# jdeschut/tunempc

Hardware: AMD Instinct MI355X
Metric: stage-Hessian convexifications/sec at (nx+nu)=32, p=64 (higher is better)
Workload: dtype f64

## Files before the change

tunempc_amd/csrc/tmpc_factor.h:

```cpp
#pragma once
#include "tmpc_common.h"

namespace tmpc {


#ifndef TMPC_LDP
#define TMPC_LDP 65
#endif
constexpr int FACT_LDS_DOUBLES = 2 * 64 * TMPC_LDP + 72 + 4 * 16 * 17 + 8;

enum { GM_SUB = 0, GM_SET = 1, GM_NEG = 2 };
constexpr int GM_NOTRI = -(1 << 30);

constexpr int SLD = 17, SUBD = 64 * SLD, SLABD = 2 * SUBD;
#ifdef TMPC_NT
#define TMPC_LD(p) __builtin_nontemporal_load(p)
#else
#define TMPC_LD(p) (*(p))
#endif
typedef const double __attribute__((address_space(1)))* gcptr;
typedef const double2_t __attribute__((address_space(1)))* gcptr2;
#define TMPC_LD4(dst, off, p, ok)                                                       \
  {                                                                                     \
    const double2_t u0_ = (ok) ? ((gcptr2)(p))[0] : (double2_t){0.0, 0.0};              \
    const double2_t u1_ = (ok) ? ((gcptr2)(p))[1] : (double2_t){0.0, 0.0};              \
    dst[(off) + 0] = u0_[0]; dst[(off) + 1] = u0_[1]; dst[(off) + 2] = u1_[0]; dst[(off) + 3] = u1_[1]; \
  }
#define TMPC_LD4F(dst, off, p, ok)                                                      \
  {                                                                                     \
    const float4_t u_ = (ok) ? *(const float4_t __attribute__((address_space(1)))*)(p) : (float4_t){0.f, 0.f, 0.f, 0.f}; \
    dst[(off) + 0] = (double)u_[0]; dst[(off) + 1] = (double)u_[1]; dst[(off) + 2] = (double)u_[2]; dst[(off) + 3] = (double)u_[3]; \
  }
typedef double __attribute__((address_space(1)))* gptr;
template <int WM, int WN, int FA, int NS = 2>
struct GemmCfg {
  static constexpr int TM = 16 * FA * WM, TN = 32 * WN, NTH = 64 * WM * WN, RP = NTH / 4;
  static constexpr int ARP = (TM + RP - 1) / RP, BRP = (TN + RP - 1) / RP;
  static constexpr int ASUB = TM * 17, BSUB = TN * 17, BUFD = NS * ASUB + NS * BSUB;
  static constexpr int LDS_DOUBLES = 2 * BUFD;
};

template <bool USE_MFMA, int WM = 2, int WN = 2, int FA = 2, int NS = 2>
__device__ __forceinline__ void wg_gemm_nt(double* C, int ldc, const double* A, int lda,
                                           const double* B, int ldb, int M, int N, int K, int mode, bool lower,
                                           double* lds) {
  typedef GemmCfg<WM, WN, FA, NS> G;
  constexpr int GKT = 16 * NS;
  constexpr int TM = G::TM, TN = G::TN, RP = G::RP, ARP = G::ARP, BRP = G::BRP, ASUB = G::ASUB, BSUB = G::BSUB, BUFD = G::BUFD;
  const int tid = threadIdx.x, lane = tid & 63, wv = tid >> 6;
  const int wr = wv / WN, wc = wv % WN;
  const int lrow = tid >> 2, lk = (tid & 3) * 4;
  const int nks = (K + GKT - 1) / GKT;
  const int fk = lane >> 4, fq = (lane >> 2) & 3, fj = lane & 3;
  const int wr0 = wr * 16 * FA, wc0 = wc * 32;
  constexpr bool CPRE = (FA <= 2) && (NS == 2);
  double acc[FA][8], cpre[CPRE ? FA : 1][8];
#pragma unroll
  for (int i = 0; i < FA; ++i)
#pragma unroll
    for (int j = 0; j < 8; ++j) { acc[i][j] = 0.0; if (CPRE) cpre[i][j] = 0.0; }
  double ra[ARP * 8], rb[BRP * 8];
  int m0 = 0, n0 = 0, ks = 0;
  const __amdgpu_buffer_rsrc_t arsrc = __builtin_amdgcn_make_buffer_rsrc((void*)A, 0, (int)(((unsigned)(M - 1) * (unsigned)lda + (unsigned)K) * 8u), 0x00020000);
  const __amdgpu_buffer_rsrc_t brsrc = __builtin_amdgcn_make_buffer_rsrc((void*)B, 0, (int)(((unsigned)(N - 1) * (unsigned)ldb + (unsigned)K) * 8u), 0x00020000);
  const unsigned avo = (unsigned)(lrow * lda + lk) * 8u, bvo = (unsigned)(lrow * ldb + lk) * 8u;
  typedef unsigned int u4_t __attribute__((ext_vector_type(4)));
#define TMPC_BLD4(dst, off, rsrc, vo, so)                                                                   \
  {                                                                                                         \
    const double2_t u0_ = __builtin_bit_cast(double2_t, __builtin_amdgcn_raw_buffer_load_b128(rsrc, (vo), (so), 0));          \
    const double2_t u1_ = __builtin_bit_cast(double2_t, __builtin_amdgcn_raw_buffer_load_b128(rsrc, (vo) + 16u, (so), 0));    \
    dst[(off) + 0] = u0_[0]; dst[(off) + 1] = u0_[1]; dst[(off) + 2] = u1_[0]; dst[(off) + 3] = u1_[1];    \
  }
#define TMPC_SLAB_LOAD(M0, N0, KN)                                                                          \
  {                                                                                                         \
    const unsigned aso = (unsigned)((M0) * lda + (KN) - lk) * 8u, bso = (unsigned)((N0) * ldb + (KN) - lk) * 8u;    \
    _Pragma("unroll") for (int rp = 0; rp < ARP; ++rp) {                                                    \
      if (RP * ARP == TM || lrow + rp * RP < TM) {                                                          \
        _Pragma("unroll") for (int h2 = 0; h2 < NS; ++h2)                                                   \
          TMPC_BLD4(ra, rp * 8 + h2 * 4, arsrc, avo + (unsigned)(rp * RP * lda + h2 * 16) * 8u, aso)        \
      }                                                                                                     \
    }                                                                                                       \
    _Pragma("unroll") for (int rp = 0; rp < BRP; ++rp) {                                                    \
      if (RP * BRP == TN || lrow + rp * RP < TN) {                                                          \
        _Pragma("unroll") for (int h2 = 0; h2 < NS; ++h2)                                                   \
          TMPC_BLD4(rb, rp * 8 + h2 * 4, brsrc, bvo + (unsigned)(rp * RP * ldb + h2 * 16) * 8u, bso)        \
      }                                                                                                     \
    }                                                                                                       \
  }
#define TMPC_SLAB_STORE(BUF)                                                                                \
  {                                                                                                         \
    double* An_ = lds + (BUF) * BUFD;                                                                       \
    double* Bn_ = An_ + NS * ASUB;                                                                           \
    _Pragma("unroll") for (int rp = 0; rp < ARP; ++rp) {                                                    \
      const int row = lrow + rp * RP;                                                                       \
      if (RP * ARP == TM || row < TM) {                                                                     \
        _Pragma("unroll") for (int h2 = 0; h2 < NS; ++h2)                                                   \
          _Pragma("unroll") for (int q = 0; q < 4; ++q) An_[h2 * ASUB + row * SLD + lk + q] = ra[rp * 8 + h2 * 4 + q]; \
      }                                                                                                     \
    }                                                                                                       \
    _Pragma("unroll") for (int rp = 0; rp < BRP; ++rp) {                                                    \
      const int row = lrow + rp * RP;                                                                       \
      if (RP * BRP == TN || row < TN) {                                                                     \
        _Pragma("unroll") for (int h2 = 0; h2 < NS; ++h2)                                                   \
          _Pragma("unroll") for (int q = 0; q < 4; ++q) Bn_[h2 * BSUB + row * SLD + lk + q] = rb[rp * 8 + h2 * 4 + q]; \
      }                                                                                                     \
    }                                                                                                       \
  }
  TMPC_SLAB_LOAD(0, 0, lk)
  __syncthreads();
  TMPC_SLAB_STORE(0)
  __syncthreads();
  int buf = 0;
  TMPC_T0()
  while (m0 < M) {
    int nm0 = m0, nn0 = n0, nks_ = ks + 1;
    if (nks_ == nks) {
      nks_ = 0; nn0 = n0 + TN;
      if (nn0 >= N || (lower && nn0 > nm0)) { nn0 = 0; nm0 = m0 + TM; }
    }
    const bool more = nm0 < M;
    if (more) TMPC_SLAB_LOAD(nm0, nn0, nks_ * GKT + lk)
    TMPC_T(0)
    const bool wave_on = (m0 + wr0 < M) && (n0 + wc0 < N) && !(lower && n0 == m0 && wc0 >= wr0 + 16 * FA);
    if (CPRE && ks == 0 && mode == GM_SUB && wave_on) {
#pragma unroll
      for (int i = 0; i < FA; ++i) {
        const int rbase = m0 + wr0 + i * 16;
#pragma unroll
        for (int m = 0; m < 2; ++m) {
          const int cbase = n0 + wc0 + m * 16;
          if (rbase < M && cbase < N) {
            gcptr2 cp2 = (gcptr2)(C + (size_t)(rbase + 4 * fq + fk) * ldc + cbase + 4 * fj);
            const double2_t u0 = cp2[0], u1 = cp2[1];
            cpre[CPRE ? i : 0][4 * m + 0] = u0[0]; cpre[CPRE ? i : 0][4 * m + 1] = u0[1]; cpre[CPRE ? i : 0][4 * m + 2] = u1[0]; cpre[CPRE ? i : 0][4 * m + 3] = u1[1];
          }
        }
      }
    }
    TMPC_T(1)
    if (wave_on) {
      const double* As = lds + buf * BUFD;
      const double* Bs = As + NS * ASUB;
      const int krem = K - ks * GKT;
      if (USE_MFMA) {
#define TMPC_MFMA_STEP(kk)                                                                              \
  {                                                                                                     \
    const int so = ((kk) & 3) * 4 + fk;                                                                 \
    const double* Ak = As + ((kk) >> 2) * ASUB + so;                                                    \
    const double* Bk = Bs + ((kk) >> 2) * BSUB + so;                                                    \
    double av[FA];                                                                                      \
    _Pragma("unroll") for (int i = 0; i < FA; ++i) av[i] = Ak[(wr0 + 16 * i + 4 * fq + fj) * SLD];       \
    _Pragma("unroll") for (int cb = 0; cb < 8; ++cb) {                                                  \
      const double bv = Bk[(wc0 + 16 * (cb >> 2) + 4 * fj + (cb & 3)) * SLD];                           \
      _Pragma("unroll") for (int i = 0; i < FA; ++i)                                                    \
        acc[i][cb] = __builtin_amdgcn_mfma_f64_4x4x4f64(av[i], bv, acc[i][cb], 0, 0, 0);                \
    }                                                                                                   \
  }
        if (NS == 1 || krem >= GKT) {
          if (FA <= 2) {
#pragma unroll
            for (int kk = 0; kk < GKT / 4; ++kk) TMPC_MFMA_STEP(kk)
          } else {
#pragma unroll 2
            for (int kk = 0; kk < GKT / 4; ++kk) TMPC_MFMA_STEP(kk)
          }
        } else {
          if (FA <= 2) {
#pragma unroll
            for (int kk = 0; kk < GKT / 8; ++kk) TMPC_MFMA_STEP(kk)
          } else {
#pragma unroll 2
            for (int kk = 0; kk < GKT / 8; ++kk) TMPC_MFMA_STEP(kk)
          }
        }
#undef TMPC_MFMA_STEP
      } else {
        const int kmax = (krem >= GKT) ? GKT : krem;
        for (int kk = 0; kk < kmax; ++kk) {
#pragma unroll
          for (int i = 0; i < FA; ++i)
#pragma unroll
            for (int cb = 0; cb < 8; ++cb) {
              const int row = wr0 + i * 16 + 4 * fq + fk, col = wc0 + 16 * (cb >> 2) + 4 * fj + (cb & 3);
              acc[i][cb] = fma(As[(kk >> 4) * ASUB + row * SLD + (kk & 15)], Bs[(kk >> 4) * BSUB + col * SLD + (kk & 15)], acc[i][cb]);
            }
        }
      }
    }
    TMPC_T(2)
    if (more) TMPC_SLAB_STORE(buf ^ 1)
    TMPC_T(3)
    if (ks == nks - 1 && wave_on) {
#pragma unroll
      for (int i = 0; i < FA; ++i) {
        const int rbase = m0 + wr0 + i * 16;
#pragma unroll
        for (int m = 0; m < 2; ++m) {
          const int cbase = n0 + wc0 + m * 16;
          if (rbase < M && cbase < N) {
            typedef double2_t __attribute__((address_space(1)))* gptr2;
            gptr2 cp2 = (gptr2)(C + (size_t)(rbase + 4 * fq + fk) * ldc + cbase + 4 * fj);
            double c0[4] = {0.0, 0.0, 0.0, 0.0};
            if (mode == GM_SUB) {
              if (CPRE) { c0[0] = cpre[CPRE ? i : 0][4 * m]; c0[1] = cpre[CPRE ? i : 0][4 * m + 1]; c0[2] = cpre[CPRE ? i : 0][4 * m + 2]; c0[3] = cpre[CPRE ? i : 0][4 * m + 3]; }
              else { const double2_t u0 = ((gcptr2)cp2)[0], u1 = ((gcptr2)cp2)[1]; c0[0] = u0[0]; c0[1] = u0[1]; c0[2] = u1[0]; c0[3] = u1[1]; }
            }
            double v[4];
#pragma unroll
            for (int e = 0; e < 4; ++e) {
              const double t = acc[i][4 * m + e];
              v[e] = (mode == GM_SUB) ? c0[e] - t : ((mode == GM_NEG) ? -t : t);
            }
            cp2[0] = (double2_t){v[0], v[1]}; cp2[1] = (double2_t){v[2], v[3]};
          }
#pragma unroll
          for (int e = 0; e < 4; ++e) acc[i][4 * m + e] = 0.0;
        }
      }
    }
    TMPC_T(4)
    __syncthreads();
    TMPC_T(5)
    buf ^= 1;
    m0 = nm0; n0 = nn0; ks = nks_;
  }
#undef TMPC_SLAB_LOAD
#undef TMPC_SLAB_STORE
#undef TMPC_BLD4
}

constexpr int LDP = TMPC_LDP;

__device__ __forceinline__ double potrf_rsqrt(double x) {
  double r = __builtin_amdgcn_rsq(x);
  r = r * (1.5 - 0.5 * x * r * r);
  r = r * (1.5 - 0.5 * x * r * r);
  return r;
}
template <int J>
__device__ __forceinline__ double row_bcast16(double v) { return __builtin_amdgcn_update_dpp(0.0, v, 0x150 + J, 0xF, 0xF, false); }
template <int K>
__device__ __forceinline__ void fmac_bcast16(double& acc, double x, double y) {
  asm volatile("s_nop 1\n\tv_fmac_f64_dpp %0, %1, %2 row_newbcast:%3 row_mask:0xf bank_mask:0xf" : "+v"(acc) : "v"(x), "v"(y), "n"(K));
}
struct Potrf16State { double a[16]; double m[4]; double nbad, minr, myref, thr8; int r, g; };
template <int J, int K>
__device__ __forceinline__ void potrf16_arow(Potrf16State& st, double nlj, double lj) {
  if constexpr (K < 16) { fmac_bcast16<K>(st.a[K], nlj, lj); potrf16_arow<J, K + 1>(st, nlj, lj); }
}
template <int J, int Q>
__device__ __forceinline__ void potrf16_mrow(Potrf16State& st, double fr) {
  if constexpr (Q <= J / 4) { fmac_bcast16<J>(st.m[Q], st.m[Q], fr); potrf16_mrow<J, Q + 1>(st, fr); }
}
template <int J>
__device__ __forceinline__ void potrf16_step(Potrf16State& st) {
  const double piv = row_bcast16<J>(st.a[J]);
  const double th8 = row_bcast16<J>(st.thr8);
  double rinv;
  {
    const double r0 = __builtin_amdgcn_rsq(piv);
    const double t = piv * r0, h = fma(-t, r0, 1.0);
    const double c = fma(0.375, h, 0.5), hc = h * c;
    rinv = fma(r0, hc, r0);
  }
  double lj = st.a[J] * rinv;
  if (__builtin_amdgcn_ballot_w64(!(piv > th8)) != 0) {
    const double ref = row_bcast16<J>(st.myref);
    if (piv < 1e-8 * ref) st.minr = fmin(st.minr, fmax(piv, 0.0) / ref);
    if (!(piv > 1e-15 * ref) || !(piv > 0.0)) {
      const double sub = (ref > 0.0 ? ref : 1.0) * 1e20;
      st.nbad += 1.0;
      rinv = potrf_rsqrt(sub);
      lj = (st.r == J) ? sub * rinv : st.a[J] * rinv;
    }
  }
  st.a[J] = lj;
  const double nlj = -lj;
  const double fr = (st.r > J) ? nlj * rinv : 0.0;
  potrf16_arow<J, J + 1>(st, nlj, lj);
  potrf16_mrow<J, 0>(st, fr);
  if constexpr (J + 1 < 16) potrf16_step<J + 1>(st);
}
template <int LDQ = LDP>
__device__ __forceinline__ void wave_potrf16(double* S, double* Si, const double* dr, double* stat, int lane) {
  Potrf16State st;
  st.r = lane & 15; st.g = lane >> 4;
#pragma unroll
  for (int k = 0; k < 16; ++k) st.a[k] = S[st.r * LDQ + k];
#pragma unroll
  for (int q = 0; q < 4; ++q) st.m[q] = (4 * q + st.g == st.r) ? 1.0 : 0.0;
  st.myref = fabs(dr[st.r]); st.thr8 = 1e-8 * st.myref;
  st.nbad = 0.0; st.minr = 1.0;
  __builtin_amdgcn_s_setprio(3);
  potrf16_step<0>(st);
  __builtin_amdgcn_s_setprio(0);
  if (lane < 16) {
#pragma unroll
    for (int k = 0; k < 16; ++k) if (k <= st.r) S[st.r * LDQ + k] = st.a[k];
  }
  wave_lds_sync();
  double myrinv;
  {
    const double d = S[st.r * LDQ + st.r];
    double x = __builtin_amdgcn_rcp(d);
    x = fma(fma(-d, x, 1.0), x, x);
    x = fma(fma(-d, x, 1.0), x, x);
    myrinv = x;
  }
#pragma unroll
  for (int q = 0; q < 4; ++q) { const int c = 4 * q + st.g; Si[st.r * LDQ + c] = (c <= st.r) ? st.m[q] * myrinv : 0.0; }
  if (lane == 0) { stat[0] += st.nbad; stat[1] = fmin(stat[1], st.minr); }
  wave_lds_sync();
}

__device__ __noinline__ int wg_potrf_inv(double* T, int ldt, double* Ti, const double* dref, int nb, double* lds, double* minr, double* stat = nullptr, int sw = 0, bool preloaded = false) {
  const int tid = threadIdx.x, lane = tid & 63, wv = tid >> 6;
  TMPC_TC0()
  double* S = lds;
  double* Si = S + 64 * LDP;
  double* dr = Si + 64 * LDP;
  double* tmp = dr + 72 + wv * (16 * 17);
  {
    const int i = tid >> 2, j0 = (tid & 3) * 16;
    double2_t v[8];
    const bool on = i < nb && j0 < nb;
    if (on && !preloaded) {
      gcptr2 src = (gcptr2)(T + (size_t)i * ldt + j0);
#pragma unroll
      for (int q = 0; q < 8; ++q) v[q] = src[q];
#pragma unroll
      for (int q = 0; q < 8; ++q) { S[i * LDP + j0 + 2 * q] = v[q][0]; S[i * LDP + j0 + 2 * q + 1] = v[q][1]; }
    }
    if (on) {
#pragma unroll
      for (int q = 0; q < 8; ++q) { Si[i * LDP + j0 + 2 * q] = 0.0; Si[i * LDP + j0 + 2 * q + 1] = 0.0; }
    }
  }
  if (tid < nb) dr[tid] = dref[tid];
  if (tid == 0) { dr[65] = 0.0; dr[66] = 1.0; }
  __syncthreads();
  const int nbk = nb >> 4;
  TMPC_TC(7, 0)
  for (int jb = 0; jb < nbk; ++jb) {
    const int o = 16 * jb;
    if (wv == sw) wave_potrf16(S + o * LDP + o, Si + o * LDP + o, dr + o, dr + 65, lane);
    __syncthreads();
    TMPC_TC(7, 1)
    {
      const int bi = jb + 1 + wv;
      if (bi < nbk) {
        double4_t acc = (double4_t){0.0, 0.0, 0.0, 0.0};
        acc = mm16(S + 16 * bi * LDP + o, LDP, Si + o * LDP + o, 1, LDP, acc, 1.0, lane);
        store_d16(S + 16 * bi * LDP + o, LDP, acc, lane);
      }
    }
    __syncthreads();
    {
      int q = 0;
      for (int bi = jb + 1; bi < nbk; ++bi)
        for (int bj = jb + 1; bj <= bi; ++bj, ++q)
          if ((q & 3) == wv) {
            double* Cp = S + 16 * bi * LDP + 16 * bj;
            double4_t acc = load_d16(Cp, LDP, lane);
            acc = mm16(S + 16 * bi * LDP + o, LDP, S + 16 * bj * LDP + o, 1, LDP, acc, -1.0, lane);
            store_d16(Cp, LDP, acc, lane);
          }
    }
    __syncthreads();
    TMPC_TC(7, 2)
  }
  for (int bi = 1; bi < nbk; ++bi) {
    const int bj = wv;
    if (bj < bi) {
      double4_t acc = (double4_t){0.0, 0.0, 0.0, 0.0};
      for (int k = bj; k < bi; ++k) acc = mm16(S + 16 * bi * LDP + 16 * k, LDP, Si + 16 * k * LDP + 16 * bj, LDP, 1, acc, 1.0, lane);
      store_d16(tmp, 17, acc, lane);
      wave_lds_sync();
      double4_t r = (double4_t){0.0, 0.0, 0.0, 0.0};
      r = mm16(Si + 16 * bi * LDP + 16 * bi, LDP, tmp, 17, 1, r, -1.0, lane);
      store_d16(Si + 16 * bi * LDP + 16 * bj, LDP, r, lane);
    }
    __syncthreads();
  }
  TMPC_TC(7, 3)
  {
    const int i = tid >> 2, j0 = (tid & 3) * 16;
    if (i < nb && j0 < nb) {
      typedef double2_t __attribute__((address_space(1)))* gptr2;
      gptr2 dt = (gptr2)(T + (size_t)i * ldt + j0);
      gptr2 di = (gptr2)(Ti + i * TB + j0);
#pragma unroll
      for (int q = 0; q < 8; ++q) {
        const int j = j0 + 2 * q;
        di[q] = (double2_t){Si[i * LDP + j], Si[i * LDP + j + 1]};
        if (j + 1 <= i) dt[q] = (double2_t){S[i * LDP + j], S[i * LDP + j + 1]};
        else if (j <= i) T[(size_t)i * ldt + j] = S[i * LDP + j];
      }
    }
  }
  __syncthreads();
  TMPC_TC(7, 4)
  const int nb_bad = (int)dr[65];
  if (stat) { if (tid == 0) { stat[0] += dr[65]; stat[1] = fmin(stat[1], dr[66]); } }
  else *minr = fmin(*minr, dr[66]);
  __syncthreads();
  return nb_bad;
}

template <bool USE_MFMA>
__device__ __forceinline__ int wg_block_column(double* Dk, double* R1, double* R2, double* Linv_k, const double* dref,
                                               int dp, double* lds, double* minr) {
  int nbad = 0;
  int jt = 0;
  TMPC_TC0()
  for (int j0 = 0; j0 < dp; j0 += TB, ++jt) {
    const int nb = (dp - j0 < TB) ? dp - j0 : TB;
    if (j0 > 0) {
      wg_gemm_nt<USE_MFMA>(Dk + (size_t)j0 * dp + j0, dp, Dk + (size_t)j0 * dp, dp, Dk + (size_t)j0 * dp, dp, dp - j0, nb, j0, GM_SUB, false, lds);
      if (R1) wg_gemm_nt<USE_MFMA>(R1 + j0, dp, R1, dp, Dk + (size_t)j0 * dp, dp, dp, nb, j0, GM_SUB, false, lds);
      if (R2) wg_gemm_nt<USE_MFMA>(R2 + j0, dp, R2, dp, Dk + (size_t)j0 * dp, dp, dp, nb, j0, GM_SUB, false, lds);
    }
    TMPC_TC(6, 0)
    double* Ti = Linv_k + (size_t)jt * TB * TB;
    nbad += wg_potrf_inv(Dk + (size_t)j0 * dp + j0, dp, Ti, dref + j0, nb, lds, minr);
    TMPC_TC(6, 1)
    if (dp - j0 - nb > 0)
      wg_gemm_nt<USE_MFMA>(Dk + (size_t)(j0 + nb) * dp + j0, dp, Dk + (size_t)(j0 + nb) * dp + j0, dp, Ti, TB, dp - j0 - nb, nb, nb, GM_SET, false, lds);
    if (R1) wg_gemm_nt<USE_MFMA>(R1 + j0, dp, R1 + j0, dp, Ti, TB, dp, nb, nb, GM_SET, false, lds);
    if (R2) wg_gemm_nt<USE_MFMA>(R2 + j0, dp, R2 + j0, dp, Ti, TB, dp, nb, nb, GM_SET, false, lds);
    TMPC_TC(6, 2)
  }
  return nbad;
}

constexpr int NCP = 4;
constexpr int GKV = 16, GLDV = GKV + 1;

template <bool TRANS, bool LOWER = false, typename MT = double>
__device__ __forceinline__ void wg_gemv16(double* Y, int yld, const double* X, int xld, const MT* M, int ldm,
                                          int rows, int cols, bool accumulate, double sgn, double* As, int nc) {
  constexpr bool F32 = sizeof(MT) == 4;
  const int tid = threadIdx.x, lane = tid & 63, wv = tid >> 6;
  const int fr = lane & 15, fk = lane >> 4;
  const int nks = cols / GKV;
  for (int m0 = 0; m0 < rows; m0 += 64) {
    double4_t acc = (double4_t){0.0, 0.0, 0.0, 0.0};
    double ra[4];
    const int lrow = TRANS ? (tid >> 4) : (tid >> 2);
    const int lcol = TRANS ? ((tid & 15) * 4) : ((tid & 3) * 4);
    const bool ok = TRANS ? (m0 + lcol < rows) : (m0 + lrow < rows);
    const MT* src = TRANS ? (M + (size_t)lrow * ldm + m0 + lcol) : (M + (size_t)(m0 + lrow) * ldm + lcol);
    const size_t kstep = TRANS ? (size_t)GKV * ldm : (size_t)GKV;
    double rb[4], rc[4], rd[4];
#define TMPC_GEMV_OK(KS) (ok && (!LOWER || (TRANS ? (m0 + lcol <= GKV * (KS) + lrow) : (GKV * (KS) + lcol <= m0 + lrow))))
#define TMPC_GEMV_LD(RG, P, OK) { if (F32) TMPC_LD4F(RG, 0, P, OK) else TMPC_LD4(RG, 0, P, OK) }
    TMPC_GEMV_LD(ra, src, TMPC_GEMV_OK(0))
    if (nks > 1) { const MT* s1 = src + kstep; TMPC_GEMV_LD(rb, s1, TMPC_GEMV_OK(1)) }
    if (nks > 2) { const MT* s1 = src + 2 * kstep; TMPC_GEMV_LD(rc, s1, TMPC_GEMV_OK(2)) }
    if (nks > 3) { const MT* s1 = src + 3 * kstep; TMPC_GEMV_LD(rd, s1, TMPC_GEMV_OK(3)) }
#define TMPC_GEMV_SLAB(RG, KS)                                                                                  \
    {                                                                                                             \
      __syncthreads();                                                                                            \
      if (TRANS) {                                                                                                \
        _Pragma("unroll") for (int q = 0; q < 4; ++q) As[(lcol + q) * GLDV + lrow] = RG[q];                     \
      } else {                                                                                                    \
        _Pragma("unroll") for (int q = 0; q < 4; ++q) As[lrow * GLDV + lcol + q] = RG[q];                       \
      }                                                                                                           \
      __syncthreads();                                                                                            \
      if ((KS) + 4 < nks) {                                                                                       \
        const MT* s2 = src + (size_t)((KS) + 4) * kstep;                                                          \
        TMPC_GEMV_LD(RG, s2, TMPC_GEMV_OK((KS) + 4))                                                             \
      }                                                                                                           \
      if (m0 + 16 * wv < rows) {                                                                                  \
        const int k0 = (KS) * GKV;                                                                                \
        _Pragma("unroll") for (int kk = 0; kk < GKV / 4; ++kk) {                                                 \
          const double a = As[(16 * wv + fr) * GLDV + kk * 4 + fk];                                               \
          const double bq = X[(fr & (NCP - 1)) * xld + k0 + kk * 4 + fk];                                         \
          acc = __builtin_amdgcn_mfma_f64_16x16x4f64(a, bq, acc, 0, 0, 0);                                        \
        }                                                                                                         \
      }                                                                                                           \
    }
    for (int ks = 0; ks < nks; ks += 4) {
      TMPC_GEMV_SLAB(ra, ks)
      if (ks + 1 < nks) TMPC_GEMV_SLAB(rb, ks + 1)
      if (ks + 2 < nks) TMPC_GEMV_SLAB(rc, ks + 2)
      if (ks + 3 < nks) TMPC_GEMV_SLAB(rd, ks + 3)
    }
#undef TMPC_GEMV_SLAB
#undef TMPC_GEMV_LD
#undef TMPC_GEMV_OK
    if (m0 + 16 * wv < rows && fr < nc) {
#pragma unroll
      for (int r = 0; r < 4; ++r) {
        const int i = m0 + 16 * wv + fk + 4 * r;
        if (i < rows) {
          double* yp = Y + fr * yld + i;
          *yp = (accumulate ? *yp : 0.0) + sgn * acc[r];
        }
      }
    }
  }
  __syncthreads();
}

__device__ __forceinline__ void blk_fwd(double* z, int xld, double* tmp, int tld, const double* Dk, const double* Lik, int dp,
                                        double* As, int nc) {
  int jt = 0;
  for (int j0 = 0; j0 < dp; j0 += TB, ++jt) {
    const int nb = (dp - j0 < TB) ? dp - j0 : TB;
    const double* Ti = Lik + (size_t)jt * TB * TB;
    wg_gemv16<false, true>(tmp, tld, z + j0, xld, Ti, TB, nb, nb, false, 1.0, As, nc);
    for (int e = threadIdx.x; e < nb * nc; e += 256) { const int q = e / nb, i = e - q * nb; z[q * xld + j0 + i] = tmp[q * tld + i]; }
    __syncthreads();
    const int rem = dp - j0 - nb;
    if (rem > 0) wg_gemv16<false>(z + j0 + nb, xld, z + j0, xld, Dk + (size_t)(j0 + nb) * dp + j0, dp, rem, nb, true, -1.0, As, nc);
  }
}
__device__ __forceinline__ void blk_bwd(double* z, int xld, double* tmp, int tld, const double* Dk, const double* Lik, int dp,
                                        double* As, int nc) {
  const int nt = (dp + TB - 1) / TB;
  for (int jt = nt - 1; jt >= 0; --jt) {
    const int j0 = jt * TB;
    const int nb = (dp - j0 < TB) ? dp - j0 : TB;
    const double* Ti = Lik + (size_t)jt * TB * TB;
    wg_gemv16<true, true>(tmp, tld, z + j0, xld, Ti, TB, nb, nb, false, 1.0, As, nc);
    for (int e = threadIdx.x; e < nb * nc; e += 256) { const int q = e / nb, i = e - q * nb; z[q * xld + j0 + i] = tmp[q * tld + i]; }
    __syncthreads();
    if (j0 > 0) wg_gemv16<true>(z, xld, z + j0, xld, Dk + (size_t)j0 * dp, dp, j0, nb, true, -1.0, As, nc);
  }
}

__device__ __forceinline__ void vec_g2s(double* z, int xld, const double* R, int dp, int nc) {
  for (int e = threadIdx.x; e < dp * nc; e += 256) { const int i = e / nc, q = e - i * nc; z[q * xld + i] = R[e]; }
}
__device__ __forceinline__ void vec_s2g(double* R, const double* z, int xld, int dp, int nc) {
  for (int e = threadIdx.x; e < dp * nc; e += 256) { const int i = e / nc, q = e - i * nc; R[e] = z[q * xld + i]; }
}

template <int NTH = 256>
__device__ __forceinline__ double wg_reduce_sum(double v, double* red) {
  const int lane = threadIdx.x & 63, wv = threadIdx.x >> 6;
  for (int o = 32; o > 0; o >>= 1) v += __shfl_xor(v, o, 64);
  __syncthreads();
  if (lane == 0) red[wv] = v;
  __syncthreads();
  double r = red[0];
#pragma unroll
  for (int q = 1; q < NTH / 64; ++q) r += red[q];
  __syncthreads();
  return r;
}

template <int NTH>
__device__ __forceinline__ void solve_border_body(const WS& w, const Dims& dm, int b, int pass, double* red) {
  const int* ip = w.iprob + (size_t)b * IS;
  const int phase = ip[I_PHASE];
  if (phase == PH_DONE) return;
  double* pr = w.prob + (size_t)b * PS;
  const int p = dm.p, dp = dm.dp, tid = threadIdx.x, nx = dm.nx;
  const size_t vl = (size_t)p * dp;
  double* W3 = w.W3 + (size_t)b * vl * 3;
  double* Z = w.Z + (size_t)b * vl;
  double* TU = w.TU + (size_t)b * vl * 2;
  const double* U = w.U + (size_t)b * vl * 2;
  if (pass == 1 && phase != PH_MAIN) return;
  const bool three = (pass == 1) || (phase != PH_MAIN && !ip[I_CHORD]);
  if (three) {
    double s00 = 0.0, s01 = 0.0, s11 = 0.0;
    for (size_t e = tid; e < vl; e += NTH) {
      const double t0 = W3[e * 3 + 1], t1 = W3[e * 3 + 2];
      TU[e * 2] = t0; TU[e * 2 + 1] = t1;
      Z[e] = W3[e * 3];
      s00 = fma(U[e * 2], t0, s00); s01 = fma(U[e * 2], t1, s01); s11 = fma(U[e * 2 + 1], t1, s11);
    }
    s00 = wg_reduce_sum<NTH>(s00, red); s01 = wg_reduce_sum<NTH>(s01, red); s11 = wg_reduce_sum<NTH>(s11, red);
    if (tid == 0) { pr[P_SB00] = pr[P_BTT] - s00; pr[P_SB01] = pr[P_BTA] - s01; pr[P_SB11] = pr[P_BAA] - s11; }
  }
  __syncthreads();
  double u0 = 0.0, u1 = 0.0;
  for (size_t e = tid; e < vl; e += NTH) { const double z = Z[e]; u0 = fma(U[e * 2], z, u0); u1 = fma(U[e * 2 + 1], z, u1); }
  u0 = wg_reduce_sum<NTH>(u0, red); u1 = wg_reduce_sum<NTH>(u1, red);
  double trt2 = 0.0, hbg = 0.0;
  for (int k = tid; k < p; k += NTH) { const double* q = w.part + (size_t)(b * p + k) * NPART; trt2 += q[Q_TRT2]; hbg += q[Q_HBG]; }
  trt2 = wg_reduce_sum<NTH>(trt2, red); hbg = wg_reduce_sum<NTH>(hbg, red);
  const double sig = (pass == 1) ? 0.0 : pr[P_SIGMU];
  const double corr0 = (pass == 1) ? 0.0 : pr[P_CORR0];
  const double s0 = pr[P_S0], x0 = pr[P_X0], rd0 = pr[P_RD0];
  const double t0 = sig / s0 - x0 * rd0 / s0 - corr0;
  const double rb0 = (trt2 - 1.0) - u0, rb1 = (hbg + t0) - u1;
  const double a = pr[P_SB00], bb = pr[P_SB01], c = pr[P_SB11];
  const double det = a * c - bb * bb;
  const double dtau = (c * rb0 - bb * rb1) / det, dalpha = (a * rb1 - bb * rb0) / det;
  __syncthreads();
  if (tid == 0) { pr[P_DTAU] = dtau; pr[P_DALPHA] = dalpha; }
  double* dPg = w.dP + (size_t)b * p * nx * nx;
  const int d = dm.d;
  for (int e = tid; e < p * d; e += NTH) {
    const int k = e / d, idx = e - k * d;
    int a2 = 0, rem = idx;
    while (rem >= nx - a2) { rem -= nx - a2; ++a2; }
    const int c2 = a2 + rem;
    const size_t vi = (size_t)k * dp + idx;
    const double v = Z[vi] - TU[vi * 2] * dtau - TU[vi * 2 + 1] * dalpha;
    dPg[(size_t)k * nx * nx + a2 * nx + c2] = v;
    dPg[(size_t)k * nx * nx + c2 * nx + a2] = v;
  }
}

__global__ void __launch_bounds__(256) k_solve_border(WS w, Dims dm, const int* alist, int pass) {
  __shared__ double red[8];
  solve_border_body<256>(w, dm, alist[blockIdx.x], pass, red);
}

}
```

Before: 12210.

## Add dedicated float32 GEMV path with 32-wide slabs and buffer loads

Adds a float32-matrix GEMV variant that stages 32-column slabs (8 floats per thread) in the fp64 LDS region and loads them with raw buffer loads, which return zero for out-of-range offsets instead of needing per-load predicates. Halving the number of slabs cuts the syncthreads pairs per K and makes each global load wider. In exchange it drops the triangular variant for float32 and depends on the buffer out-of-bounds behaviour for masking, including a sentinel offset for inactive lanes.

```diff
diff --git a/tunempc_amd/csrc/tmpc_factor.h b/tunempc_amd/csrc/tmpc_factor.h
--- a/tunempc_amd/csrc/tmpc_factor.h
+++ b/tunempc_amd/csrc/tmpc_factor.h
@@ -25,11 +25,6 @@
     const double2_t u0_ = (ok) ? ((gcptr2)(p))[0] : (double2_t){0.0, 0.0};              \
     const double2_t u1_ = (ok) ? ((gcptr2)(p))[1] : (double2_t){0.0, 0.0};              \
     dst[(off) + 0] = u0_[0]; dst[(off) + 1] = u0_[1]; dst[(off) + 2] = u1_[0]; dst[(off) + 3] = u1_[1]; \
-  }
-#define TMPC_LD4F(dst, off, p, ok)                                                      \
-  {                                                                                     \
-    const float4_t u_ = (ok) ? *(const float4_t __attribute__((address_space(1)))*)(p) : (float4_t){0.f, 0.f, 0.f, 0.f}; \
-    dst[(off) + 0] = (double)u_[0]; dst[(off) + 1] = (double)u_[1]; dst[(off) + 2] = (double)u_[2]; dst[(off) + 3] = (double)u_[3]; \
   }
 typedef double __attribute__((address_space(1)))* gptr;
 template <int WM, int WN, int FA, int NS = 2>
@@ -436,10 +431,91 @@
 constexpr int NCP = 4;
 constexpr int GKV = 16, GLDV = GKV + 1;
 
+constexpr int GKF = 32, GLDF = GKF + 1;
+static_assert(64 * GLDF * sizeof(float) <= 64 * GLDV * sizeof(double), "the float32 slab lives in the As region of the fp64 form");
+template <bool TRANS>
+__device__ __forceinline__ void wg_gemv32f(double* Y, int yld, const double* X, int xld, const float* M, int ldm,
+                                           int rows, int cols, bool accumulate, double sgn, double* As, int nc) {
+  float* Af = (float*)As;
+  const int tid = threadIdx.x, lane = tid & 63, wv = tid >> 6;
+  const int fr = lane & 15, fk = lane >> 4;
+  const int nks = (cols + GKF - 1) / GKF;
+  const unsigned mbytes = TRANS ? ((unsigned)(cols - 1) * (unsigned)ldm + (unsigned)rows) * 4u : (unsigned)rows * (unsigned)ldm * 4u;
+  const __amdgpu_buffer_rsrc_t mrsrc = __builtin_amdgcn_make_buffer_rsrc((void*)M, 0, (int)mbytes, 0x00020000);
+  const unsigned kstep = (TRANS ? (unsigned)GKF * (unsigned)ldm : (unsigned)GKF) * 4u;
+  const unsigned piece = (TRANS ? 16u * (unsigned)ldm : 4u) * 4u;
+  typedef unsigned int u4_t __attribute__((ext_vector_type(4)));
+  for (int m0 = 0; m0 < rows; m0 += 64) {
+    double4_t acc = (double4_t){0.0, 0.0, 0.0, 0.0};
+    const int lrow = TRANS ? (tid >> 4) : (tid >> 2);
+    const int lcol = TRANS ? ((tid & 15) * 4) : ((tid & 3) * 8);
+    const unsigned vo = TRANS ? ((m0 + lcol < rows) ? ((unsigned)lrow * (unsigned)ldm + (unsigned)(m0 + lcol)) * 4u : 0x40000000u)
+                              : ((unsigned)(m0 + lrow) * (unsigned)ldm + (unsigned)lcol) * 4u;
+    float ra[8], rb[8], rc[8], rd[8];
+#define TMPC_GEMV_LD(RG, KS)                                                                                      \
+    {                                                                                                             \
+      const unsigned o_ = vo + (unsigned)(KS) * kstep;                                                            \
+      const float4_t u0_ = __builtin_bit_cast(float4_t, __builtin_amdgcn_raw_buffer_load_b128(mrsrc, (int)o_, 0, 0));           \
+      const float4_t u1_ = __builtin_bit_cast(float4_t, __builtin_amdgcn_raw_buffer_load_b128(mrsrc, (int)(o_ + piece), 0, 0)); \
+      _Pragma("unroll") for (int q = 0; q < 4; ++q) { RG[q] = u0_[q]; RG[4 + q] = u1_[q]; }                     \
+    }
+    TMPC_GEMV_LD(ra, 0)
+    if (nks > 1) TMPC_GEMV_LD(rb, 1)
+    if (nks > 2) TMPC_GEMV_LD(rc, 2)
+    if (nks > 3) TMPC_GEMV_LD(rd, 3)
+#define TMPC_GEMV_MFMA4(KK0)                                                                                      \
+        _Pragma("unroll") for (int kk = (KK0); kk < (KK0) + 4; ++kk) {                                           \
+          const double a = (double)Af[(16 * wv + fr) * GLDF + kk * 4 + fk];                                       \
+          const double bq = X[(fr & (NCP - 1)) * xld + k0 + kk * 4 + fk];                                         \
+          acc = __builtin_amdgcn_mfma_f64_16x16x4f64(a, bq, acc, 0, 0, 0);                                        \
+        }
+#define TMPC_GEMV_SLAB(RG, KS)                                                                                  \
+    {                                                                                                             \
+      __syncthreads();                                                                                            \
+      if (TRANS) {                                                                                                \
+        _Pragma("unroll") for (int q = 0; q < 4; ++q) { Af[(lcol + q) * GLDF + lrow] = RG[q]; Af[(lcol + q) * GLDF + 16 + lrow] = RG[4 + q]; } \
+      } else {                                                                                                    \
+        _Pragma("unroll") for (int q = 0; q < 8; ++q) Af[lrow * GLDF + lcol + q] = RG[q];                       \
+      }                                                                                                           \
+      __syncthreads();                                                                                            \
+      if ((KS) + 4 < nks) TMPC_GEMV_LD(RG, (KS) + 4)                                                              \
+      if (m0 + 16 * wv < rows) {                                                                                  \
+        const int k0 = (KS) * GKF;                                                                                \
+        TMPC_GEMV_MFMA4(0)                                                                                        \
+        if (k0 + 16 < cols) { TMPC_GEMV_MFMA4(4) }                                                                \
+      }                                                                                                           \
+    }
+    for (int ks = 0; ks < nks; ks += 4) {
+      TMPC_GEMV_SLAB(ra, ks)
+      if (ks + 1 < nks) TMPC_GEMV_SLAB(rb, ks + 1)
+      if (ks + 2 < nks) TMPC_GEMV_SLAB(rc, ks + 2)
+      if (ks + 3 < nks) TMPC_GEMV_SLAB(rd, ks + 3)
+    }
+#undef TMPC_GEMV_SLAB
+#undef TMPC_GEMV_MFMA4
+#undef TMPC_GEMV_LD
+    if (m0 + 16 * wv < rows && fr < nc) {
+#pragma unroll
+      for (int r = 0; r < 4; ++r) {
+        const int i = m0 + 16 * wv + fk + 4 * r;
+        if (i < rows) {
+          double* yp = Y + fr * yld + i;
+          *yp = (accumulate ? *yp : 0.0) + sgn * acc[r];
+        }
+      }
+    }
+  }
+  __syncthreads();
+}
+
 template <bool TRANS, bool LOWER = false, typename MT = double>
 __device__ __forceinline__ void wg_gemv16(double* Y, int yld, const double* X, int xld, const MT* M, int ldm,
                                           int rows, int cols, bool accumulate, double sgn, double* As, int nc) {
-  constexpr bool F32 = sizeof(MT) == 4;
+  if constexpr (sizeof(MT) == 4) {
+    static_assert(!LOWER, "the float32 form has no triangular variant");
+    wg_gemv32f<TRANS>(Y, yld, X, xld, M, ldm, rows, cols, accumulate, sgn, As, nc);
+    return;
+  }
   const int tid = threadIdx.x, lane = tid & 63, wv = tid >> 6;
   const int fr = lane & 15, fk = lane >> 4;
   const int nks = cols / GKV;
@@ -453,7 +529,7 @@
     const size_t kstep = TRANS ? (size_t)GKV * ldm : (size_t)GKV;
     double rb[4], rc[4], rd[4];
 #define TMPC_GEMV_OK(KS) (ok && (!LOWER || (TRANS ? (m0 + lcol <= GKV * (KS) + lrow) : (GKV * (KS) + lcol <= m0 + lrow))))
-#define TMPC_GEMV_LD(RG, P, OK) { if (F32) TMPC_LD4F(RG, 0, P, OK) else TMPC_LD4(RG, 0, P, OK) }
+#define TMPC_GEMV_LD(RG, P, OK) TMPC_LD4(RG, 0, P, OK)
     TMPC_GEMV_LD(ra, src, TMPC_GEMV_OK(0))
     if (nks > 1) { const MT* s1 = src + kstep; TMPC_GEMV_LD(rb, s1, TMPC_GEMV_OK(1)) }
     if (nks > 2) { const MT* s1 = src + 2 * kstep; TMPC_GEMV_LD(rc, s1, TMPC_GEMV_OK(2)) }
```

After: 12470, median of 6. +2.1%, better.
